# intelligent-machine-learning/dlrover

Hardware: AMD Instinct MI355X
Metric: checkpoint save+restore sec and goodput % under injected failure, Llama-3-8B FSDP 1/2/4/8 MI355X (higher is better)
Workload: dtype bf16; 1 GPU; model=llama3_8b, params=8030261248, global_batch=2, seq_len=4096, parallelism=fsdp1, ckpt_interval=2, ckpt_scope=full, ckpt_restored_step=1

## Files before the change

### dlrover_amd/ops/csrc/attention_bwd_v3.hip

```cpp
#include <cstdlib>
#include "kern_common.h"

typedef __attribute__((ext_vector_type(8))) __bf16 bf16x8;
typedef __attribute__((ext_vector_type(16))) float f32x16_t;
typedef __attribute__((ext_vector_type(2))) unsigned int u32x2_t;
typedef __attribute__((ext_vector_type(4))) unsigned int u32x4_t;
typedef __attribute__((ext_vector_type(2))) __bf16 bf16x2;

#define FB_D 128
#define FB_QB 256
#define FB_T 64

__device__ __forceinline__ int swzb(int row, int byte_col) {
  return byte_col ^ ((row & 7) << 4);
}

__device__ __forceinline__ unsigned pk_bf16(float lo, float hi) {
  bf16x2 v = {(__bf16)lo, (__bf16)hi};
  return *reinterpret_cast<unsigned*>(&v);
}

__device__ __forceinline__ bf16x8 trT_frag(const char* lds, int rb, int n,
                                           int lane, int half) {
  const int j = (lane & 15) >> 2;
  const int dq = n * 8 + ((lane & 16) >> 2) + (lane & 3);
  const int r0 = rb + half * 8 + j;
  const int r1 = r0 + 4;
  const unsigned base = (unsigned)(uintptr_t)lds;
  const unsigned a0 = base + r0 * 256 + ((dq * 8) ^ ((r0 & 7) << 4));
  const unsigned a1 = base + r1 * 256 + ((dq * 8) ^ ((r1 & 7) << 4));
  u32x2_t w0, w1;
  asm volatile(
      "ds_read_b64_tr_b16 %0, %2\n\t"
      "ds_read_b64_tr_b16 %1, %3\n\t"
      "s_waitcnt lgkmcnt(0)"
      : "=v"(w0), "=v"(w1)
      : "v"(a0), "v"(a1));
  u32x4_t frag = u32x4_t{w0.x, w0.y, w1.x, w1.y};
  return *reinterpret_cast<bf16x8*>(&frag);
}

__device__ __forceinline__ void pairswap_frags(const float v16[16], int half,
                                               bf16x8 out[2]) {
#pragma unroll
  for (int ks2 = 0; ks2 < 2; ++ks2) {
    const int r0 = ks2 * 8;
    unsigned w0 = pk_bf16(v16[r0 + 0], v16[r0 + 1]);
    unsigned w1 = pk_bf16(v16[r0 + 2], v16[r0 + 3]);
    unsigned w2 = pk_bf16(v16[r0 + 4], v16[r0 + 5]);
    unsigned w3 = pk_bf16(v16[r0 + 6], v16[r0 + 7]);
    u32x2_t s0 = __builtin_amdgcn_permlane32_swap(w0, w2, false, false);
    u32x2_t s1 = __builtin_amdgcn_permlane32_swap(w1, w3, false, false);
    u32x4_t frag = u32x4_t{s0.x, s1.x, s0.y, s1.y};
    out[ks2] = *reinterpret_cast<bf16x8*>(&frag);
  }
  (void)half;
}


__global__ __launch_bounds__(512) void fa_bwd_dq_v3_kernel(
    const short* __restrict__ q, const short* __restrict__ k,
    const short* __restrict__ v, const short* __restrict__ dout,
    const float* __restrict__ lse, const float* __restrict__ dvec,
    short* __restrict__ dq, int B, int H, int HKV, int S, float scale,
    long long qs_b, long long qs_h, long long qs_s,
    long long ks_b, long long ks_h, long long ks_s,
    long long vs_b, long long vs_h, long long vs_s,
    long long ds_b, long long ds_h, long long ds_s) {
  __shared__ char k_lds[2][FB_T * FB_D * 2];
  __shared__ char v_lds[2][FB_T * FB_D * 2];

  const int tid = threadIdx.x;
  const int wave = tid >> 6;
  const int lane = tid & 63;
  const int half = lane >> 5;
  const int qcol = lane & 31;

  const int qt = blockIdx.x;
  const int h = blockIdx.y;
  const int b = blockIdx.z;
  const int g = h / (H / HKV);

  const short* q_blk = q + (long long)b * qs_b + (long long)h * qs_h +
                       (long long)(qt * FB_QB) * qs_s;
  const short* do_blk = dout + (long long)b * ds_b + (long long)h * ds_h +
                        (long long)(qt * FB_QB) * ds_s;
  const short* k_head = k + (long long)b * ks_b + (long long)g * ks_h;
  const short* v_head = v + (long long)b * vs_b + (long long)g * vs_h;

  const int q_row_w = wave * 32 + qcol;
  const int q_glob = qt * FB_QB + q_row_w;

  bf16x8 bq[8], bdo[8];
#pragma unroll
  for (int ks = 0; ks < 8; ++ks) {
    bq[ks] = *reinterpret_cast<const bf16x8*>(
        q_blk + (long long)q_row_w * qs_s + ks * 16 + half * 8);
    bdo[ks] = *reinterpret_cast<const bf16x8*>(
        do_blk + (long long)q_row_w * ds_s + ks * 16 + half * 8);
  }
  const long long lrow = ((long long)b * H + h) * S + q_glob;
  const float L = lse[lrow];
  const float Dv = dvec[lrow];

  f32x16_t acc_dq[4];
#pragma unroll
  for (int n = 0; n < 4; ++n)
#pragma unroll
    for (int r = 0; r < 16; ++r) acc_dq[n][r] = 0.f;

  bf16x8 st_k[2], st_v[2];
  const int st_row0 = (tid * 16) / FB_D;
  const int st_col0 = (tid * 16) % FB_D;
  auto issue_loads = [&](int kt) {
    const short* ksrc = k_head + (long long)(kt * FB_T) * ks_s;
    const short* vsrc = v_head + (long long)(kt * FB_T) * vs_s;
#pragma unroll
    for (int c = 0; c < 2; ++c) {
      st_k[c] = *reinterpret_cast<const bf16x8*>(
          ksrc + (long long)st_row0 * ks_s + st_col0 + c * 8);
      st_v[c] = *reinterpret_cast<const bf16x8*>(
          vsrc + (long long)st_row0 * vs_s + st_col0 + c * 8);
    }
  };
  auto write_lds = [&](int buf) {
#pragma unroll
    for (int c = 0; c < 2; ++c) {
      const int col = st_col0 + c * 8;
      *reinterpret_cast<bf16x8*>(k_lds[buf] + st_row0 * 256 +
                                 swzb(st_row0, col * 2)) = st_k[c];
      *reinterpret_cast<bf16x8*>(v_lds[buf] + st_row0 * 256 +
                                 swzb(st_row0, col * 2)) = st_v[c];
    }
  };

  const int n_tiles = (qt + 1) * (FB_QB / FB_T);
  const int wave_q_max = qt * FB_QB + wave * 32 + 31;

  issue_loads(0);
  write_lds(0);
  __syncthreads();

  for (int kt = 0; kt < n_tiles; ++kt) {
    const int cur = kt & 1;
    const char* k_cur = k_lds[cur];
    const char* v_cur = v_lds[cur];
    if (kt + 1 < n_tiles) issue_loads(kt + 1);

    const int kv0 = kt * FB_T;
    if (kv0 <= wave_q_max) {
      bf16x8 bds[4];
#pragma unroll
      for (int n = 0; n < 2; ++n) {
        f32x16_t acc_s;
#pragma unroll
        for (int r = 0; r < 16; ++r) acc_s[r] = 0.f;
#pragma unroll
        for (int ks = 0; ks < 8; ++ks) {
          const int row = n * 32 + qcol;
          bf16x8 ak = *reinterpret_cast<const bf16x8*>(
              k_cur + row * 256 + swzb(row, (ks * 16 + half * 8) * 2));
          acc_s = __builtin_amdgcn_mfma_f32_32x32x16_bf16(ak, bq[ks], acc_s,
                                                          0, 0, 0);
        }
#pragma unroll
        for (int r = 0; r < 16; ++r) {
          const int kv_glob = kv0 + n * 32 + (r & 3) + 8 * (r >> 2) + 4 * half;
          acc_s[r] =
              (kv_glob > q_glob) ? 0.f : __expf(acc_s[r] * scale - L);
        }
        f32x16_t acc_dp;
#pragma unroll
        for (int r = 0; r < 16; ++r) acc_dp[r] = 0.f;
#pragma unroll
        for (int ks = 0; ks < 8; ++ks) {
          const int row = n * 32 + qcol;
          bf16x8 av = *reinterpret_cast<const bf16x8*>(
              v_cur + row * 256 + swzb(row, (ks * 16 + half * 8) * 2));
          acc_dp = __builtin_amdgcn_mfma_f32_32x32x16_bf16(av, bdo[ks],
                                                           acc_dp, 0, 0, 0);
        }
        float dsv[16];
#pragma unroll
        for (int r = 0; r < 16; ++r)
          dsv[r] = acc_s[r] * (acc_dp[r] - Dv) * scale;
        pairswap_frags(dsv, half, &bds[n * 2]);
      }
#pragma unroll
      for (int n = 0; n < 4; ++n) {
#pragma unroll
        for (int ks = 0; ks < 4; ++ks) {
          bf16x8 akT = trT_frag(k_cur, ks * 16, n, lane, half);
          acc_dq[n] = __builtin_amdgcn_mfma_f32_32x32x16_bf16(
              akT, bds[ks], acc_dq[n], 0, 0, 0);
        }
      }
    }

    __syncthreads();
    if (kt + 1 < n_tiles) {
      write_lds(cur ^ 1);
      __syncthreads();
    }
  }

  short* dq_blk = dq + (long long)b * qs_b + (long long)h * qs_h +
                  (long long)(qt * FB_QB) * qs_s;
  char* slab = (char*)k_lds + (wave & 3) * (32 * FB_D * 2);
  for (int round = 0; round < 2; ++round) {
    __syncthreads();
    if ((wave >> 2) == round) {
#pragma unroll
      for (int n = 0; n < 4; ++n) {
#pragma unroll
        for (int r = 0; r < 16; ++r) {
          const int d = n * 32 + (r & 3) + 8 * (r >> 2) + 4 * half;
          *reinterpret_cast<__bf16*>(slab + qcol * 256 + swzb(qcol, d * 2)) =
              (__bf16)acc_dq[n][r];
        }
      }
    }
    __syncthreads();
    if ((wave >> 2) == round) {
#pragma unroll
      for (int pass = 0; pass < 4; ++pass) {
        const int elem0 = (pass * 64 + lane) * 16;
        const int r2 = elem0 / FB_D;
        const int c2 = elem0 % FB_D;
        bf16x8 v0 = *reinterpret_cast<const bf16x8*>(
            slab + r2 * 256 + swzb(r2, c2 * 2));
        bf16x8 v1 = *reinterpret_cast<const bf16x8*>(
            slab + r2 * 256 + swzb(r2, (c2 + 8) * 2));
        short* dst = dq_blk + (long long)(wave * 32 + r2) * qs_s + c2;
        *reinterpret_cast<bf16x8*>(dst) = v0;
        *reinterpret_cast<bf16x8*>(dst + 8) = v1;
      }
    }
  }
}


#define FB_DKV_PROLOGUE()                                                    \
  __shared__ char q_lds[FB_T * FB_D * 2];                                    \
  __shared__ char do_lds[FB_T * FB_D * 2];                                   \
  __shared__ float l_lds[FB_T];                                              \
  __shared__ float d_lds[FB_T];                                              \
  const int tid = threadIdx.x;                                               \
  const int wave = tid >> 6;                                                 \
  const int lane = tid & 63;                                                 \
  const int half = lane >> 5;                                                \
  const int kcol = lane & 31;                                                \
  const int kvb0 = blockIdx.x * FB_QB;                                       \
  const int chunk = blockIdx.y;                                              \
  const int CH = gridDim.y;                                                  \
  const int bg = blockIdx.z;                                                 \
  const int b = bg / HKV;                                                    \
  const int g = bg % HKV;                                                    \
  const int rep = H / HKV;                                                   \
  const int kv_own = kvb0 + wave * 32 + kcol;                                \
  const short* k_head = k + (long long)b * ks_b + (long long)g * ks_h;       \
  bf16x8 bk[8];                                                              \
  _Pragma("unroll") for (int ks = 0; ks < 8; ++ks) bk[ks] =                  \
      *reinterpret_cast<const bf16x8*>(k_head + (long long)kv_own * ks_s +   \
                                       ks * 16 + half * 8);                  \
  const int qt_min = kvb0 / FB_T;                                            \
  const int n_qt = S / FB_T - qt_min;                                        \
  const int n_work = rep * n_qt;                                             \
  const int wave_kv_min = kvb0 + wave * 32;                                  \
  auto stage_qdo = [&](int h, int qt) {                                      \
    const short* qsrc = q + (long long)b * qs_b + (long long)h * qs_h +      \
                        (long long)(qt * FB_T) * qs_s;                       \
    const short* dsrc = dout + (long long)b * ds_b + (long long)h * ds_h +   \
                        (long long)(qt * FB_T) * ds_s;                       \
    _Pragma("unroll") for (int c = 0; c < 2; ++c) {                          \
      const int linear = (tid * 16) + c * 8;                                 \
      const int row = linear / FB_D;                                         \
      const int col = linear % FB_D;                                         \
      *reinterpret_cast<bf16x8*>(q_lds + row * 256 + swzb(row, col * 2)) =   \
          *reinterpret_cast<const bf16x8*>(qsrc + (long long)row * qs_s +    \
                                           col);                             \
      *reinterpret_cast<bf16x8*>(do_lds + row * 256 + swzb(row, col * 2)) =  \
          *reinterpret_cast<const bf16x8*>(dsrc + (long long)row * ds_s +    \
                                           col);                             \
    }                                                                        \
    if (tid < FB_T) {                                                        \
      const long long lrow = ((long long)b * H + h) * S + qt * FB_T + tid;   \
      l_lds[tid] = lse[lrow];                                                \
      d_lds[tid] = dvec[lrow];                                               \
    }                                                                        \
  }

__global__ __launch_bounds__(512) void fa_bwd_dv_v3_kernel(
    const short* __restrict__ q, const short* __restrict__ k,
    const short* __restrict__ v, const short* __restrict__ dout,
    const float* __restrict__ lse, const float* __restrict__ dvec,
    float* __restrict__ dk32, float* __restrict__ dv32, int B, int H,
    int HKV, int S, float scale,
    long long qs_b, long long qs_h, long long qs_s,
    long long ks_b, long long ks_h, long long ks_s,
    long long vs_b, long long vs_h, long long vs_s,
    long long ds_b, long long ds_h, long long ds_s) {
  FB_DKV_PROLOGUE();

  {
    f32x16_t acc_dv[4];
#pragma unroll
    for (int n = 0; n < 4; ++n)
#pragma unroll
      for (int r = 0; r < 16; ++r) acc_dv[n][r] = 0.f;

    for (int w = chunk; w < n_work; w += CH) {
      const int h = g * rep + w / n_qt;
      const int qt = qt_min + w % n_qt;
      __syncthreads();
      stage_qdo(h, qt);
      __syncthreads();
      if (qt * FB_T + FB_T - 1 < wave_kv_min) continue;
#pragma unroll
      for (int st = 0; st < 2; ++st) {
        const int q0 = qt * FB_T + st * 32;
        if (q0 + 31 < wave_kv_min) continue;
        f32x16_t acc_s;
#pragma unroll
        for (int r = 0; r < 16; ++r) acc_s[r] = 0.f;
#pragma unroll
        for (int ks = 0; ks < 8; ++ks) {
          const int row = st * 32 + kcol;
          bf16x8 aq = *reinterpret_cast<const bf16x8*>(
              q_lds + (st * 32 + kcol) * 256 +
              swzb(st * 32 + kcol, (ks * 16 + half * 8) * 2));
          (void)row;
          acc_s = __builtin_amdgcn_mfma_f32_32x32x16_bf16(aq, bk[ks], acc_s,
                                                          0, 0, 0);
        }
        float pv[16];
#pragma unroll
        for (int r = 0; r < 16; ++r) {
          const int qrow = st * 32 + (r & 3) + 8 * (r >> 2) + 4 * half;
          const int q_glob = qt * FB_T + qrow;
          pv[r] = (kv_own > q_glob)
                      ? 0.f
                      : __expf(acc_s[r] * scale - l_lds[qrow]);
        }
        bf16x8 bp[2];
        pairswap_frags(pv, half, bp);
#pragma unroll
        for (int n = 0; n < 4; ++n) {
#pragma unroll
          for (int ks2 = 0; ks2 < 2; ++ks2) {
            bf16x8 adoT =
                trT_frag(do_lds, st * 32 + ks2 * 16, n, lane, half);
            acc_dv[n] = __builtin_amdgcn_mfma_f32_32x32x16_bf16(
                adoT, bp[ks2], acc_dv[n], 0, 0, 0);
          }
        }
      }
    }
    float* dv_base = dv32 + ((long long)bg * S + kv_own) * FB_D;
#pragma unroll
    for (int n = 0; n < 4; ++n)
// ... 140 lines not shown
```

### dlrover_amd/ops/csrc/bindings.cpp

```cpp
#include <torch/extension.h>
#include <ATen/cuda/CUDAContext.h>

#include <tuple>

extern "C" {
void rmsnorm_fwd_launch(const void*, const void*, void*, void*, int, int,
                        float, void*);
void rmsnorm_add_fwd_launch(const void*, const void*, const void*, void*,
                            void*, void*, int, int, float, void*);
void rmsnorm_bwd_launch(const void*, const void*, const void*, const void*,
                        const void*, void*, void*, void*, void*, int, int,
                        int, void*);
void rope_launch(void*, const void*, const void*, const void*, long long,
                 long long, int, int, int, void*);
void rope_oop_launch(const void*, void*, const void*, const void*,
                     const void*, long long, long long, int, int, long long,
                     int, void*);
void swiglu_fwd_launch(const void*, void*, long long, int, void*);
void swiglu_bwd_launch(const void*, const void*, void*, long long, int, void*);
void adamw_launch(void*, const void*, void*, void*, void*, long long, float,
                  float, float, float, float, int, int, float, void*);
void causal_softmax_fwd_launch(void*, long long, int, int, int, float, void*);
void causal_softmax_bwd_launch(void*, const void*, long long, int, float,
                               void*);
void cross_entropy_launch(void*, const void*, void*, long long, int, int,
                          float, int, void*);
void mfma16_probe_launch(const void*, const void*, void*, void*);
void mfma32_probe_launch(const void*, const void*, void*, void*);
void tr_b16_probe3_launch(void*, void*);
void tr_b16_probe_launch(void*, void*);
void flash_attn_fwd_launch(const void*, const void*, const void*, void*,
                           void*, int, int, int, int, float,
                           const long long*, void*);
void flash_attn_fwd_v3_launch(const void*, const void*, const void*, void*,
                              void*, int, int, int, int, float,
                              const long long*, void*);
void flash_attn_fwd_v2_launch(const void*, const void*, const void*, void*,
                              void*, int, int, int, int, float,
                              const long long*, void*);
void fa_bwd_pre_launch(const void*, const void*, void*, int, int, int,
                       const long long*, const long long*, void*);
void fa_bwd_dq_launch(const void*, const void*, const void*, const void*,
                      const void*, const void*, void*, int, int, int, int,
                      float, const long long*, void*);
void fa_bwd_dq_v3_launch(const void*, const void*, const void*, const void*,
                         const void*, const void*, void*, int, int, int, int,
                         float, const long long*, void*);
void fa_bwd_dkv_v3_launch(const void*, const void*, const void*, const void*,
                          const void*, const void*, void*, void*, int, int,
                          int, int, float, const long long*, void*);
void fa_bwd_dkv_launch(const void*, const void*, const void*, const void*,
                       const void*, const void*, void*, void*, int, int, int,
                       int, float, const long long*, void*);
void f32_to_bf16_launch(const void*, void*, long long, void*);
}

namespace {

void* cur_stream() {
  return (void*)at::cuda::getCurrentCUDAStream().stream();
}

void check_bf16(const at::Tensor& t, const char* name) {
  TORCH_CHECK(t.is_cuda(), name, " must be on GPU");
  TORCH_CHECK(t.is_contiguous(), name, " must be contiguous");
  TORCH_CHECK(t.scalar_type() == at::kBFloat16, name, " must be bf16");
}

std::tuple<at::Tensor, at::Tensor> rmsnorm_fwd(const at::Tensor& x,
                                               const at::Tensor& w,
                                               double eps) {
  check_bf16(x, "x");
  check_bf16(w, "w");
  const int hidden = (int)x.size(-1);
  TORCH_CHECK(hidden % 8 == 0, "hidden must be a multiple of 8");
  const long long n_rows = x.numel() / hidden;
  auto y = at::empty_like(x);
  auto invrms = at::empty({n_rows}, x.options().dtype(at::kFloat));
  rmsnorm_fwd_launch(x.data_ptr(), w.data_ptr(), y.data_ptr(),
                     invrms.data_ptr(), (int)n_rows, hidden, (float)eps,
                     cur_stream());
  return {y, invrms};
}

std::tuple<at::Tensor, at::Tensor, at::Tensor> rmsnorm_add_fwd(
    const at::Tensor& x, const at::Tensor& resid, const at::Tensor& w,
    double eps) {
  check_bf16(x, "x");
  check_bf16(resid, "resid");
  const int hidden = (int)x.size(-1);
  const long long n_rows = x.numel() / hidden;
  auto h = at::empty_like(x);
  auto y = at::empty_like(x);
  auto invrms = at::empty({n_rows}, x.options().dtype(at::kFloat));
  rmsnorm_add_fwd_launch(x.data_ptr(), resid.data_ptr(), w.data_ptr(),
                         h.data_ptr(), y.data_ptr(), invrms.data_ptr(),
                         (int)n_rows, hidden, (float)eps, cur_stream());
  return {h, y, invrms};
}

std::tuple<at::Tensor, at::Tensor> rmsnorm_bwd(
    const at::Tensor& dy, const at::Tensor& x, const at::Tensor& w,
    const at::Tensor& invrms, c10::optional<at::Tensor> dh_extra) {
  check_bf16(dy, "dy");
  check_bf16(x, "x");
  const int hidden = (int)x.size(-1);
  TORCH_CHECK(hidden <= 16384, "rmsnorm_bwd: hidden > 16384 unsupported "
              "(register dw accumulator: RMSN_MAX_VPT)");
  const long long n_rows = x.numel() / hidden;
  const int n_partials = (int)(n_rows < 2048 ? (n_rows > 0 ? n_rows : 1) : 2048);
  auto dx = at::empty_like(x);
  auto dw = at::empty_like(w);
  auto partial =
      at::empty({n_partials, hidden}, x.options().dtype(at::kFloat));
  auto dw_f32 = at::zeros({hidden}, x.options().dtype(at::kFloat));
  const void* dh_ptr = nullptr;
  if (dh_extra.has_value()) {
    check_bf16(*dh_extra, "dh_extra");
    dh_ptr = dh_extra->data_ptr();
  }
  rmsnorm_bwd_launch(dy.data_ptr(), x.data_ptr(), w.data_ptr(),
                     invrms.data_ptr(), dh_ptr, dx.data_ptr(),
                     partial.data_ptr(), dw_f32.data_ptr(), dw.data_ptr(),
                     (int)n_rows, hidden, n_partials, cur_stream());
  return {dx, dw};
}

void rope_apply(at::Tensor& x, const at::Tensor& pos, const at::Tensor& cos,
                const at::Tensor& sin, bool backward) {
  check_bf16(x, "x");
  TORCH_CHECK(pos.scalar_type() == at::kInt && pos.is_cuda(),
              "pos must be int32 on GPU");
  TORCH_CHECK(cos.scalar_type() == at::kFloat && cos.is_contiguous(),
              "cos table must be contiguous fp32");
  const int head_dim = (int)x.size(-1);
  const int n_heads = (int)x.size(-2);
  TORCH_CHECK(head_dim % 8 == 0, "head_dim must be a multiple of 8");
  const long long n_tokens = x.numel() / ((long long)n_heads * head_dim);
  TORCH_CHECK(pos.numel() > 0 && n_tokens % pos.numel() == 0,
              "pos length must divide the token count (one entry per "
              "sequence position)");
  rope_launch(x.data_ptr(), pos.data_ptr(), cos.data_ptr(), sin.data_ptr(),
              n_tokens, (long long)pos.numel(), n_heads, head_dim,
              backward ? 1 : 0, cur_stream());
}

at::Tensor rope_rotate_oop(const at::Tensor& x, const at::Tensor& pos,
                           const at::Tensor& cos, const at::Tensor& sin,
                           bool backward) {
  TORCH_CHECK(x.is_cuda(), "x must be on GPU");
  TORCH_CHECK(x.scalar_type() == at::kBFloat16, "x must be bf16");
  TORCH_CHECK(pos.scalar_type() == at::kInt && pos.is_cuda(),
              "pos must be int32 on GPU");
  const int head_dim = (int)x.size(-1);
  const int n_heads = (int)x.size(-2);
  TORCH_CHECK(head_dim % 8 == 0, "head_dim must be a multiple of 8");
  TORCH_CHECK(x.stride(-1) == 1 && x.stride(-2) == head_dim,
              "rope: head_dim/heads must be contiguous within a token row");
  const long long n_tokens = x.numel() / ((long long)n_heads * head_dim);
  long long tok_stride = n_heads * (long long)head_dim;
  if (x.dim() >= 3) {
    tok_stride = x.stride(-3);
    long long rows = x.size(-3);
    for (int d = (int)x.dim() - 4; d >= 0; --d) {
      TORCH_CHECK(x.stride(d) == rows * tok_stride,
                  "rope: leading dims must be uniformly strided");
      rows *= x.size(d);
    }
  }
  TORCH_CHECK(pos.numel() > 0 && n_tokens % pos.numel() == 0,
              "pos length must divide the token count");
  auto out = at::empty(x.sizes(), x.options());
  rope_oop_launch(x.data_ptr(), out.data_ptr(), pos.data_ptr(),
                  cos.data_ptr(), sin.data_ptr(), n_tokens,
                  (long long)pos.numel(), n_heads, head_dim, tok_stride,
                  backward ? 1 : 0, cur_stream());
  return out;
}

at::Tensor swiglu_fwd(const at::Tensor& gate_up) {
  check_bf16(gate_up, "gate_up");
  const int two_inner = (int)gate_up.size(-1);
  TORCH_CHECK(two_inner % 16 == 0, "inner dim must be a multiple of 8");
  const int inner = two_inner / 2;
  const long long n_rows = gate_up.numel() / two_inner;
  auto sizes = gate_up.sizes().vec();
  sizes.back() = inner;
  auto out = at::empty(sizes, gate_up.options());
  swiglu_fwd_launch(gate_up.data_ptr(), out.data_ptr(), n_rows, inner,
                    cur_stream());
  return out;
}

at::Tensor swiglu_bwd(const at::Tensor& dy, const at::Tensor& gate_up) {
  check_bf16(dy, "dy");
  check_bf16(gate_up, "gate_up");
  const int inner = (int)gate_up.size(-1) / 2;
  const long long n_rows = gate_up.numel() / (2LL * inner);
  auto d_gate_up = at::empty_like(gate_up);
  swiglu_bwd_launch(dy.data_ptr(), gate_up.data_ptr(), d_gate_up.data_ptr(),
                    n_rows, inner, cur_stream());
  return d_gate_up;
}

void adamw_step(at::Tensor& param, const at::Tensor& grad, at::Tensor& m,
                at::Tensor& v, c10::optional<at::Tensor> param_bf16,
                double lr, double beta1, double beta2, double eps,
                double weight_decay, int64_t step, double grad_scale) {
  TORCH_CHECK(param.scalar_type() == at::kFloat && param.is_contiguous(),
              "master param must be contiguous fp32");
  TORCH_CHECK(grad.is_cuda() && grad.is_contiguous(), "grad must be GPU");
  TORCH_CHECK(grad.numel() == param.numel(), "grad/param numel mismatch");
  const bool gbf16 = grad.scalar_type() == at::kBFloat16;
  TORCH_CHECK(gbf16 || grad.scalar_type() == at::kFloat,
              "grad must be bf16 or fp32");
  void* pb = nullptr;
  if (param_bf16.has_value()) {
    check_bf16(*param_bf16, "param_bf16");
    pb = param_bf16->data_ptr();
  }
  adamw_launch(param.data_ptr(), grad.data_ptr(), m.data_ptr(), v.data_ptr(),
               pb, param.numel(), (float)lr, (float)beta1, (float)beta2,
               (float)eps, (float)weight_decay, (int)step, gbf16 ? 1 : 0,
               (float)grad_scale, cur_stream());
}

void causal_softmax_fwd(at::Tensor& scores, int64_t q_len, int64_t q_offset,
                        double scale) {
  check_bf16(scores, "scores");
  const int row_len = (int)scores.size(-1);
  TORCH_CHECK(row_len % 8 == 0, "row_len must be a multiple of 8");
  const long long n_rows = scores.numel() / row_len;
  causal_softmax_fwd_launch(scores.data_ptr(), n_rows, row_len, (int)q_len,
                            (int)q_offset, (float)scale, cur_stream());
}

void causal_softmax_bwd(at::Tensor& dscores, const at::Tensor& probs,
                        double scale) {
  check_bf16(dscores, "dscores");
  check_bf16(probs, "probs");
  const int row_len = (int)dscores.size(-1);
  const long long n_rows = dscores.numel() / row_len;
  causal_softmax_bwd_launch(dscores.data_ptr(), probs.data_ptr(), n_rows,
                            row_len, (float)scale, cur_stream());
}

static void check_attn_view(const at::Tensor& t, const char* name) {
  TORCH_CHECK(t.is_cuda() && t.scalar_type() == at::kBFloat16, name,
              " must be bf16 GPU");
  TORCH_CHECK(t.dim() == 4 && t.stride(3) == 1, name,
              " must be [B,H,S,D] with contiguous D");
}

static void pack_strides(long long* st, const at::Tensor& t, int at) {
  st[at + 0] = (long long)t.stride(0);
  st[at + 1] = (long long)t.stride(1);
  st[at + 2] = (long long)t.stride(2);
}

std::tuple<at::Tensor, at::Tensor> flash_attn_fwd(const at::Tensor& q,
                                                  const at::Tensor& k,
                                                  const at::Tensor& v,
                                                  double scale) {
  check_attn_view(q, "q");
  check_attn_view(k, "k");
  check_attn_view(v, "v");
  const int B = (int)q.size(0), H = (int)q.size(1), S = (int)q.size(2);
  const int D = (int)q.size(3), HKV = (int)k.size(1);
  TORCH_CHECK(D == 128, "flash_attn: head_dim must be 128");
  TORCH_CHECK(S % 64 == 0, "flash_attn: seq len must be a multiple of 64");
  TORCH_CHECK(H % HKV == 0, "flash_attn: H % HKV != 0");
  auto out_bshd = at::empty({B, S, H, D}, q.options());
  auto out = out_bshd.permute({0, 2, 1, 3});
  auto lse = at::empty({B, H, S}, q.options().dtype(at::kFloat));
  long long st[12];
  pack_strides(st, q, 0);
  pack_strides(st, k, 3);
  pack_strides(st, v, 6);
  pack_strides(st, out, 9);
  static const bool use_v2 = []() {
    const char* e = getenv("DLROVER_FA_V2");
    return e != nullptr && e[0] == '1';
  }();
  static const bool v3_enabled = []() {
    const char* e = getenv("DLROVER_FA_V3");
    return e == nullptr || e[0] != '0';
  }();
  if (v3_enabled && !use_v2 && S % 256 == 0) {
    flash_attn_fwd_v3_launch(q.data_ptr(), k.data_ptr(), v.data_ptr(),
                             out_bshd.data_ptr(), lse.data_ptr(), B, H, HKV,
                             S, (float)scale, st, cur_stream());
  } else if (use_v2) {
    flash_attn_fwd_v2_launch(q.data_ptr(), k.data_ptr(), v.data_ptr(),
                             out_bshd.data_ptr(), lse.data_ptr(), B, H, HKV,
                             S, (float)scale, st, cur_stream());
  } else {
    flash_attn_fwd_launch(q.data_ptr(), k.data_ptr(), v.data_ptr(),
                          out_bshd.data_ptr(), lse.data_ptr(), B, H, HKV, S,
                          (float)scale, st, cur_stream());
  }
  return {out, lse};
}

std::tuple<at::Tensor, at::Tensor, at::Tensor> flash_attn_bwd(
    const at::Tensor& q, const at::Tensor& k, const at::Tensor& v,
    const at::Tensor& out, const at::Tensor& dout_in, const at::Tensor& lse,
    double scale) {
  check_attn_view(q, "q");
  check_attn_view(k, "k");
  check_attn_view(v, "v");
  const int B = (int)q.size(0), H = (int)q.size(1), S = (int)q.size(2);
  const int D = (int)q.size(3), HKV = (int)k.size(1);
  at::Tensor dout = dout_in;
  if (dout.strides() != out.strides()) {
    dout = at::empty_like(out.permute({0, 2, 1, 3}).contiguous())
               .view({B, S, H, D});
    dout = dout.permute({0, 2, 1, 3});
    dout.copy_(dout_in);
  }
  TORCH_CHECK(dout.stride(3) == 1, "dout needs contiguous D");
  auto dvec = at::empty({B, H, S}, q.options().dtype(at::kFloat));
  {
    long long ost[3], dstr[3];
    pack_strides(ost, out, 0);
    pack_strides(dstr, dout, 0);
    fa_bwd_pre_launch(dout.data_ptr(), out.data_ptr(), dvec.data_ptr(), B, H,
                      S, ost, dstr, cur_stream());
    long long st[12];
    pack_strides(st, q, 0);
    pack_strides(st, k, 3);
    pack_strides(st, v, 6);
    pack_strides(st, dout, 9);
    auto dq_bshd = at::empty({B, S, H, D}, q.options());
    auto dq = dq_bshd.permute({0, 2, 1, 3});
    {
      long long stq[12];
      pack_strides(stq, dq, 0);
      pack_strides(stq, k, 3);
      pack_strides(stq, v, 6);
      pack_strides(stq, dout, 9);
      at::Tensor quse = q;
      if (q.strides() != dq.strides()) {
        auto q_bshd = at::empty({B, S, H, D}, q.options());
        auto qv = q_bshd.permute({0, 2, 1, 3});
        qv.copy_(q);
        quse = qv;
        pack_strides(stq, quse, 0);
      }
      static const bool bwd_v3 = []() {
        const char* e = getenv("DLROVER_FA_BWD_V3");
        return e == nullptr || e[0] != '0';
      }();
      auto dk32 = at::zeros({B, HKV, S, D}, k.options().dtype(at::kFloat));
      auto dv32 = at::zeros({B, HKV, S, D}, v.options().dtype(at::kFloat));
      if (bwd_v3 && S % 256 == 0) {
        fa_bwd_dq_v3_launch(quse.data_ptr(), k.data_ptr(), v.data_ptr(),
                            dout.data_ptr(), lse.data_ptr(), dvec.data_ptr(),
                            dq_bshd.data_ptr(), B, H, HKV, S, (float)scale,
                            stq, cur_stream());
        fa_bwd_dkv_v3_launch(quse.data_ptr(), k.data_ptr(), v.data_ptr(),
                             dout.data_ptr(), lse.data_ptr(),
                             dvec.data_ptr(), dk32.data_ptr(),
                             dv32.data_ptr(), B, H, HKV, S, (float)scale,
                             stq, cur_stream());
      } else {
        fa_bwd_dq_launch(quse.data_ptr(), k.data_ptr(), v.data_ptr(),
                         dout.data_ptr(), lse.data_ptr(), dvec.data_ptr(),
                         dq_bshd.data_ptr(), B, H, HKV, S, (float)scale, stq,
                         cur_stream());
        fa_bwd_dkv_launch(quse.data_ptr(), k.data_ptr(), v.data_ptr(),
                          dout.data_ptr(), lse.data_ptr(), dvec.data_ptr(),
                          dk32.data_ptr(), dv32.data_ptr(), B, H, HKV, S,
                          (float)scale, stq, cur_stream());
      }
      auto dk = at::empty({B, HKV, S, D}, k.options());
      auto dv = at::empty({B, HKV, S, D}, v.options());
      f32_to_bf16_launch(dk32.data_ptr(), dk.data_ptr(), dk32.numel(),
                         cur_stream());
      f32_to_bf16_launch(dv32.data_ptr(), dv.data_ptr(), dv32.numel(),
                         cur_stream());
      return {dq, dk, dv};
    }
  }
}

at::Tensor mfma16_probe(const at::Tensor& A, const at::Tensor& B) {
  check_bf16(A, "A");
  check_bf16(B, "B");
  TORCH_CHECK(A.sizes() == at::IntArrayRef({16, 32}) &&
              B.sizes() == at::IntArrayRef({32, 16}),
              "probe wants A[16,32], B[32,16]");
  auto C = at::empty({16, 16}, A.options().dtype(at::kFloat));
  mfma16_probe_launch(A.data_ptr(), B.data_ptr(), C.data_ptr(), cur_stream());
  return C;
}

void memcpy_d2h_async(int64_t dst_addr, const at::Tensor& src) {
  TORCH_CHECK(src.is_cuda() && src.is_contiguous(), "src must be cuda+contig");
  auto err = hipMemcpyAsync((void*)dst_addr, src.data_ptr(), src.nbytes(),
                            hipMemcpyDeviceToHost,
                            (hipStream_t)cur_stream());
  TORCH_CHECK(err == hipSuccess, "hipMemcpyAsync D2H: ", hipGetErrorString(err));
}

void memcpy_h2d_async(at::Tensor& dst, int64_t src_addr, int64_t nbytes) {
  TORCH_CHECK(dst.is_cuda() && dst.is_contiguous(), "dst must be cuda+contig");
  TORCH_CHECK(nbytes <= (int64_t)dst.nbytes(), "overflow");
  auto err = hipMemcpyAsync(dst.data_ptr(), (const void*)src_addr, nbytes,
                            hipMemcpyHostToDevice,
                            (hipStream_t)cur_stream());
  TORCH_CHECK(err == hipSuccess, "hipMemcpyAsync H2D: ", hipGetErrorString(err));
}

at::Tensor mfma32_probe(const at::Tensor& A, const at::Tensor& B) {
  check_bf16(A, "A");
  check_bf16(B, "B");
  TORCH_CHECK(A.sizes() == at::IntArrayRef({32, 16}) &&
              B.sizes() == at::IntArrayRef({16, 32}),
              "probe wants A[32,16], B[16,32]");
  auto C = at::empty({32, 32}, A.options().dtype(at::kFloat));
  mfma32_probe_launch(A.data_ptr(), B.data_ptr(), C.data_ptr(), cur_stream());
  return C;
}

at::Tensor cross_entropy_fwd_bwd(at::Tensor& logits, const at::Tensor& targets,
                                 int64_t ignore_index, double grad_scale,
                                 bool compute_grad) {
  check_bf16(logits, "logits");
  TORCH_CHECK(targets.scalar_type() == at::kInt && targets.is_cuda(),
              "targets must be int32 on GPU");
  const int vocab = (int)logits.size(-1);
  const long long n_rows = logits.numel() / vocab;
  TORCH_CHECK(targets.numel() == n_rows, "one target per row");
  auto losses = at::empty({n_rows}, logits.options().dtype(at::kFloat));
  cross_entropy_launch(logits.data_ptr(), targets.data_ptr(),
                       losses.data_ptr(), n_rows, vocab, (int)ignore_index,
                       (float)grad_scale, compute_grad ? 1 : 0, cur_stream());
  return losses;
}

}

PYBIND11_MODULE(TORCH_EXTENSION_NAME, m) {
  m.doc() = "dlrover_amd CDNA4 (gfx950) kernels";
  m.def("rmsnorm_fwd", &rmsnorm_fwd, "fused RMSNorm forward (bf16)");
  m.def("rmsnorm_bwd", &rmsnorm_bwd, "fused RMSNorm backward (bf16)");
  m.def("rmsnorm_add_fwd", &rmsnorm_add_fwd,
        "fused residual-add + RMSNorm forward -> (h, y, invrms)");
  m.def("rope_apply", &rope_apply, "in-place RoPE rotate-half (bf16)");
  m.def("rope_rotate_oop", &rope_rotate_oop,
        "out-of-place RoPE: strided source -> contiguous output");
  m.def("swiglu_fwd", &swiglu_fwd, "fused SwiGLU forward (bf16)");
  m.def("swiglu_bwd", &swiglu_bwd, "fused SwiGLU backward (bf16)");
  m.def("adamw_step", &adamw_step, "fused AdamW with fp32 master weights");
  m.def("causal_softmax_fwd", &causal_softmax_fwd,
        "in-place fused scale+causal-mask+softmax (bf16)");
  m.def("causal_softmax_bwd", &causal_softmax_bwd,
        "in-place softmax backward (bf16)");
  m.def("cross_entropy_fwd_bwd", &cross_entropy_fwd_bwd,
        "fused CE loss + in-place dlogits (bf16)");
  m.def("tr_b16_probe", []() {
    auto out = at::empty({64, 12}, at::TensorOptions()
                                      .dtype(at::kBFloat16)
                                      .device(at::kCUDA));
    tr_b16_probe_launch(out.data_ptr(), cur_stream());
    return out;
  }, "ds_read_b64_tr_b16 semantics probe");
  m.def("mfma16_probe", &mfma16_probe, "MFMA 16x16x32 bf16 layout self-test");
  m.def("mfma32_probe", &mfma32_probe, "MFMA 32x32x16 bf16 layout self-test");
  m.def("memcpy_d2h_async", &memcpy_d2h_async,
        "hipMemcpyAsync device tensor -> registered host address");
  m.def("memcpy_h2d_async", &memcpy_h2d_async,
        "hipMemcpyAsync registered host address -> device tensor");
  m.def("tr_b16_probe3", []() {
    auto out = at::empty({64, 12}, at::TensorOptions()
                                      .dtype(at::kShort)
                                      .device(at::kCUDA));
    tr_b16_probe3_launch(out.data_ptr(), cur_stream());
    return out;
  }, "tr_b16 cooperative tile-sourcing probe (raw index bits)");
  m.def("flash_attn_fwd", &flash_attn_fwd,
        "flash attention forward (bf16, causal, GQA, D=128) -> (out, lse)");
  m.def("flash_attn_bwd", &flash_attn_bwd,
        "flash attention backward -> (dq, dk, dv)");
}
```

### setup.py

```python

import os

from setuptools import setup

os.environ.setdefault("PYTORCH_ROCM_ARCH", "gfx950")

from torch.utils.cpp_extension import BuildExtension, CUDAExtension

ROOT = os.path.dirname(os.path.abspath(__file__))
CSRC = os.path.join(ROOT, "dlrover_amd", "ops", "csrc")

sources = [
    os.path.join(CSRC, "bindings.cpp"),
    os.path.join(CSRC, "rmsnorm.hip"),
    os.path.join(CSRC, "rope.hip"),
    os.path.join(CSRC, "swiglu.hip"),
    os.path.join(CSRC, "adamw.hip"),
    os.path.join(CSRC, "softmax.hip"),
    os.path.join(CSRC, "cross_entropy.hip"),
    os.path.join(CSRC, "mfma_probe.hip"),
    os.path.join(CSRC, "attention.hip"),
    os.path.join(CSRC, "attention_v3.hip"),
    os.path.join(CSRC, "attention_bwd.hip"),
    os.path.join(CSRC, "attention_bwd_v3.hip"),
]

setup(
    name="dlrover_amd_ops",
    ext_modules=[
        CUDAExtension(
            name="dlrover_amd.ops._hip_ops",
            sources=sources,
            extra_compile_args={
                "cxx": ["-O3", "-std=c++17"],
                "nvcc": ["-O3", "-std=c++17", "--offload-arch=gfx950"],
            },
        )
    ],
    cmdclass={"build_ext": BuildExtension.with_options(use_ninja=True)},
)
```

Measured before the change: 60.07 goodput_percent.

## Add v4 flash-attention dK/dV backward kernel with balanced chunking and direct bf16 output

Adds a new dK/dV backward kernel that splits work across blocks in load-balanced chunks sized to the CU count. It double-buffers Q/dO tiles in LDS and writes bf16 dK/dV directly when a key block is not chunked, which avoids the fp32 zero-init, atomics and conversion pass in that case. Chunked key blocks still use fp32 atomics plus a conversion kernel. The code becomes the default through a new variant argument, and the shared fragment helpers move into a common header. The metric is checkpoint goodput, so changes in backward attention time may barely show up in it.

```diff
diff --git a/dlrover_amd/ops/csrc/attention_bwd_v3.hip b/dlrover_amd/ops/csrc/attention_bwd_v3.hip
--- a/dlrover_amd/ops/csrc/attention_bwd_v3.hip
+++ b/dlrover_amd/ops/csrc/attention_bwd_v3.hip
@@ -1,61 +1,5 @@
 #include <cstdlib>
-#include "kern_common.h"
-
-typedef __attribute__((ext_vector_type(8))) __bf16 bf16x8;
-typedef __attribute__((ext_vector_type(16))) float f32x16_t;
-typedef __attribute__((ext_vector_type(2))) unsigned int u32x2_t;
-typedef __attribute__((ext_vector_type(4))) unsigned int u32x4_t;
-typedef __attribute__((ext_vector_type(2))) __bf16 bf16x2;
-
-#define FB_D 128
-#define FB_QB 256
-#define FB_T 64
-
-__device__ __forceinline__ int swzb(int row, int byte_col) {
-  return byte_col ^ ((row & 7) << 4);
-}
-
-__device__ __forceinline__ unsigned pk_bf16(float lo, float hi) {
-  bf16x2 v = {(__bf16)lo, (__bf16)hi};
-  return *reinterpret_cast<unsigned*>(&v);
-}
-
-__device__ __forceinline__ bf16x8 trT_frag(const char* lds, int rb, int n,
-                                           int lane, int half) {
-  const int j = (lane & 15) >> 2;
-  const int dq = n * 8 + ((lane & 16) >> 2) + (lane & 3);
-  const int r0 = rb + half * 8 + j;
-  const int r1 = r0 + 4;
-  const unsigned base = (unsigned)(uintptr_t)lds;
-  const unsigned a0 = base + r0 * 256 + ((dq * 8) ^ ((r0 & 7) << 4));
-  const unsigned a1 = base + r1 * 256 + ((dq * 8) ^ ((r1 & 7) << 4));
-  u32x2_t w0, w1;
-  asm volatile(
-      "ds_read_b64_tr_b16 %0, %2\n\t"
-      "ds_read_b64_tr_b16 %1, %3\n\t"
-      "s_waitcnt lgkmcnt(0)"
-      : "=v"(w0), "=v"(w1)
-      : "v"(a0), "v"(a1));
-  u32x4_t frag = u32x4_t{w0.x, w0.y, w1.x, w1.y};
-  return *reinterpret_cast<bf16x8*>(&frag);
-}
-
-__device__ __forceinline__ void pairswap_frags(const float v16[16], int half,
-                                               bf16x8 out[2]) {
-#pragma unroll
-  for (int ks2 = 0; ks2 < 2; ++ks2) {
-    const int r0 = ks2 * 8;
-    unsigned w0 = pk_bf16(v16[r0 + 0], v16[r0 + 1]);
-    unsigned w1 = pk_bf16(v16[r0 + 2], v16[r0 + 3]);
-    unsigned w2 = pk_bf16(v16[r0 + 4], v16[r0 + 5]);
-    unsigned w3 = pk_bf16(v16[r0 + 6], v16[r0 + 7]);
-    u32x2_t s0 = __builtin_amdgcn_permlane32_swap(w0, w2, false, false);
-    u32x2_t s1 = __builtin_amdgcn_permlane32_swap(w1, w3, false, false);
-    u32x4_t frag = u32x4_t{s0.x, s1.x, s0.y, s1.y};
-    out[ks2] = *reinterpret_cast<bf16x8*>(&frag);
-  }
-  (void)half;
-}
+#include "fa_bwd_frag.h"
 
 
 __global__ __launch_bounds__(512) void fa_bwd_dq_v3_kernel(
diff --git a/dlrover_amd/ops/csrc/attention_bwd_v4.hip b/dlrover_amd/ops/csrc/attention_bwd_v4.hip
--- /dev/null
+++ b/dlrover_amd/ops/csrc/attention_bwd_v4.hip
@@ -0,0 +1,337 @@
+#include "fa_bwd_frag.h"
+
+#define F4_QDO_BYTES (2 * 2 * FB_T * FB_D * 2)
+#define F4_VIMG_BYTES (FB_QB * FB_D * 2)
+#define F4_LD_BYTES (2 * 2 * FB_T * 4)
+#define F4_SMEM (F4_QDO_BYTES + F4_VIMG_BYTES + F4_LD_BYTES)
+#define F4_NUM_CU 256
+#define F4_MIN_UNITS 8
+
+__host__ __device__ __forceinline__ int f4_nch(int n_work, int T) {
+  return (n_work + T - 1) / T;
+}
+
+static int f4_units_per_item(int B, int H, int HKV, int S) {
+  const int rep = H / HKV;
+  long long total = 0;
+  for (int kb = 0; kb < S / FB_QB; ++kb)
+    total += (long long)rep * (S / FB_T - kb * (FB_QB / FB_T));
+  total *= (long long)B * HKV;
+  long long T = (total + 2 * F4_NUM_CU - 1) / (2 * F4_NUM_CU);
+  return T < F4_MIN_UNITS ? F4_MIN_UNITS : (int)T;
+}
+
+__device__ __forceinline__ int f4_slab_pos(int row, int d) {
+  return row * FB_D + (d ^ (row & 31) ^ (((d >> 2) & 1) << 5));
+}
+
+template <int OFF0, int OFF1>
+__device__ __forceinline__ bf16x8 f4_tr(unsigned addr) {
+  u32x2_t w0, w1;
+  asm volatile(
+      "ds_read_b64_tr_b16 %0, %2 offset:%3\n\t"
+      "ds_read_b64_tr_b16 %1, %2 offset:%4\n\t"
+      "s_waitcnt lgkmcnt(0)"
+      : "=&v"(w0), "=&v"(w1)
+      : "v"(addr), "n"(OFF0), "n"(OFF1));
+  u32x4_t frag = u32x4_t{w0.x, w0.y, w1.x, w1.y};
+  return *reinterpret_cast<bf16x8*>(&frag);
+}
+
+template <int ST>
+__device__ __forceinline__ void f4_accum(unsigned tile, const bf16x8 (&bp)[2],
+                                         const bf16x8 (&bds)[2],
+                                         f32x16_t (&acc_dv)[4],
+                                         f32x16_t (&acc_dk)[4]) {
+#define F4_STEP(N, KS2)                                                      \
+  {                                                                          \
+    constexpr int o0 = (ST * 32 + KS2 * 16) * 256 + N * 64;                  \
+    constexpr int o1 = (ST * 32 + KS2 * 16) * 256 + (N ^ 1) * 64 + 1024;     \
+    constexpr int dO = FB_T * FB_D * 2;                                      \
+    bf16x8 adoT = f4_tr<o0 + dO, o1 + dO>(tile);                             \
+    acc_dv[N] = __builtin_amdgcn_mfma_f32_32x32x16_bf16(adoT, bp[KS2],       \
+                                                        acc_dv[N], 0, 0, 0); \
+    bf16x8 aqT = f4_tr<o0, o1>(tile);                                        \
+    acc_dk[N] = __builtin_amdgcn_mfma_f32_32x32x16_bf16(aqT, bds[KS2],       \
+                                                        acc_dk[N], 0, 0, 0); \
+  }
+  F4_STEP(0, 0) F4_STEP(0, 1) F4_STEP(1, 0) F4_STEP(1, 1)
+  F4_STEP(2, 0) F4_STEP(2, 1) F4_STEP(3, 0) F4_STEP(3, 1)
+#undef F4_STEP
+}
+
+__global__ __launch_bounds__(512) void fa_bwd_dkv_v4_kernel(
+    const short* __restrict__ q, const short* __restrict__ k,
+    const short* __restrict__ v, const short* __restrict__ dout,
+    const float* __restrict__ lse, const float* __restrict__ dvec,
+    float* __restrict__ dk32, float* __restrict__ dv32,
+    short* __restrict__ dk, short* __restrict__ dv, int B, int H, int HKV,
+    int S, float scale, int T,
+    long long qs_b, long long qs_h, long long qs_s,
+    long long ks_b, long long ks_h, long long ks_s,
+    long long vs_b, long long vs_h, long long vs_s,
+    long long ds_b, long long ds_h, long long ds_s) {
+  __shared__ __attribute__((aligned(16))) char smem[F4_SMEM];
+  char* const qdo_lds = smem;
+  char* const v_img = smem + F4_QDO_BYTES;
+  float* const ld_lds =
+      reinterpret_cast<float*>(smem + F4_QDO_BYTES + F4_VIMG_BYTES);
+
+  const int tid = threadIdx.x;
+  const int wave = tid >> 6;
+  const int lane = tid & 63;
+  const int half = lane >> 5;
+  const int kcol = lane & 31;
+
+  const int rep = H / HKV;
+  const int BG = B * HKV;
+  const int nkb = S / FB_QB;
+  int idx = blockIdx.x, kb = 0, nch = 1;
+  for (; kb < nkb; ++kb) {
+    nch = f4_nch(rep * (S / FB_T - kb * (FB_QB / FB_T)), T);
+    const int cnt = nch * BG;
+    if (idx < cnt) break;
+    idx -= cnt;
+  }
+  if (kb >= nkb) return;
+  const int chunk = idx / BG;
+  const int bg = idx % BG;
+  const int b = bg / HKV;
+  const int g = bg % HKV;
+  const int kvb0 = kb * FB_QB;
+  const int kv_own = kvb0 + wave * 32 + kcol;
+  const int qt_min = kvb0 / FB_T;
+  const int n_qt = S / FB_T - qt_min;
+  const int n_work = rep * n_qt;
+  const int wave_kv_min = kvb0 + wave * 32;
+  const int tr_j = (lane & 15) >> 2;
+  const int tr_dql = ((lane & 16) >> 2) + (lane & 3);
+  const unsigned tr_lane_off =
+      (half * 8 + tr_j) * 256 + ((tr_dql * 8) ^ (tr_j << 4));
+
+  const short* k_head = k + (long long)b * ks_b + (long long)g * ks_h;
+  bf16x8 bk[8];
+#pragma unroll
+  for (int ks = 0; ks < 8; ++ks)
+    bk[ks] = *reinterpret_cast<const bf16x8*>(
+        k_head + (long long)kv_own * ks_s + ks * 16 + half * 8);
+
+  {
+    const short* v_rows = v + (long long)b * vs_b + (long long)g * vs_h +
+                          (long long)wave_kv_min * vs_s;
+#pragma unroll
+    for (int i = 0; i < 8; ++i) {
+      const int linear = (i * 64 + lane) * 8;
+      const int row = linear / FB_D;
+      const int col = linear % FB_D;
+      *reinterpret_cast<bf16x8*>(v_img + (wave * 32 + row) * 256 +
+                                 swzb(row, col * 2)) =
+          *reinterpret_cast<const bf16x8*>(v_rows + (long long)row * vs_s +
+                                           col);
+    }
+  }
+  const char* const v_wave = v_img + wave * 32 * 256;
+  int rd_off[4];
+#pragma unroll
+  for (int i = 0; i < 4; ++i)
+    rd_off[i] = kcol * 256 + swzb(kcol, (i * 16 + half * 8) * 2);
+
+  f32x16_t acc_dv[4], acc_dk[4];
+#pragma unroll
+  for (int n = 0; n < 4; ++n)
+#pragma unroll
+    for (int r = 0; r < 16; ++r) acc_dv[n][r] = acc_dk[n][r] = 0.f;
+
+  bf16x8 st_x[2];
+  float st_c = 0.f;
+  const int st_row = tid >> 3;
+  const int st_col = (tid & 7) * 16;
+  auto issue_loads = [&](int w, int which) {
+    const int h = g * rep + w / n_qt;
+    const int qt = qt_min + w % n_qt;
+    const short* src =
+        which ? dout + (long long)b * ds_b + (long long)h * ds_h +
+                    (long long)(qt * FB_T + st_row) * ds_s + st_col
+              : q + (long long)b * qs_b + (long long)h * qs_h +
+                    (long long)(qt * FB_T + st_row) * qs_s + st_col;
+#pragma unroll
+    for (int c = 0; c < 2; ++c)
+      st_x[c] = *reinterpret_cast<const bf16x8*>(src + c * 8);
+    if (tid < FB_T) {
+      const long long lrow = ((long long)b * H + h) * S + qt * FB_T + tid;
+      st_c = which ? dvec[lrow] : lse[lrow];
+    }
+  };
+  auto commit_lds = [&](int buf, int which) {
+    char* xb = qdo_lds + (buf * 2 + which) * (FB_T * FB_D * 2);
+#pragma unroll
+    for (int c = 0; c < 2; ++c)
+      *reinterpret_cast<bf16x8*>(
+          xb + st_row * 256 + swzb(st_row, (st_col + c * 8) * 2)) = st_x[c];
+    if (tid < FB_T)
+      ld_lds[(buf * 2 + which) * FB_T + tid] = st_c;
+  };
+
+  issue_loads(chunk, 0);
+  commit_lds(0, 0);
+  issue_loads(chunk, 1);
+  commit_lds(0, 1);
+  __syncthreads();
+
+  int cur = 0;
+  for (int w = chunk; w < n_work; w += nch) {
+    const int qt = qt_min + w % n_qt;
+    const bool more = w + nch < n_work;
+
+    const char* q_lds = qdo_lds + cur * (2 * FB_T * FB_D * 2);
+    const char* do_lds = q_lds + FB_T * FB_D * 2;
+    const float* l_lds = ld_lds + cur * 2 * FB_T;
+    const float* d_lds = l_lds + FB_T;
+
+    const bool live = qt * FB_T + FB_T - 1 >= wave_kv_min;
+#pragma unroll
+    for (int st = 0; st < 2; ++st) {
+      if (more) issue_loads(w + nch, st);
+      const int q0 = qt * FB_T + st * 32;
+      if (live && q0 + 31 >= wave_kv_min) {
+        f32x16_t acc_s, acc_dp;
+#pragma unroll
+        for (int r = 0; r < 16; ++r) acc_s[r] = acc_dp[r] = 0.f;
+#pragma unroll
+        for (int ks = 0; ks < 8; ++ks) {
+          const int ro = rd_off[ks & 3] + (ks >> 2) * 128;
+          bf16x8 aq = *reinterpret_cast<const bf16x8*>(
+              q_lds + st * (32 * 256) + ro);
+          acc_s = __builtin_amdgcn_mfma_f32_32x32x16_bf16(aq, bk[ks], acc_s,
+                                                          0, 0, 0);
+          bf16x8 ado = *reinterpret_cast<const bf16x8*>(
+              do_lds + st * (32 * 256) + ro);
+          bf16x8 bv = *reinterpret_cast<const bf16x8*>(v_wave + ro);
+          acc_dp = __builtin_amdgcn_mfma_f32_32x32x16_bf16(ado, bv, acc_dp,
+                                                           0, 0, 0);
+        }
+        float pv[16], dsv[16];
+#pragma unroll
+        for (int r = 0; r < 16; ++r) {
+          const int qrow = st * 32 + (r & 3) + 8 * (r >> 2) + 4 * half;
+          const int q_glob = qt * FB_T + qrow;
+          const float p = (kv_own > q_glob)
+                              ? 0.f
+                              : __expf(acc_s[r] * scale - l_lds[qrow]);
+          pv[r] = p;
+          dsv[r] = p * (acc_dp[r] - d_lds[qrow]) * scale;
+        }
+        bf16x8 bp[2], bds[2];
+        pairswap_frags(pv, half, bp);
+        pairswap_frags(dsv, half, bds);
+        const unsigned tile = (unsigned)(uintptr_t)q_lds + tr_lane_off;
+        if (st == 0)
+          f4_accum<0>(tile, bp, bds, acc_dv, acc_dk);
+        else
+          f4_accum<1>(tile, bp, bds, acc_dv, acc_dk);
+      }
+      if (more) commit_lds(cur ^ 1, st);
+    }
+    __syncthreads();
+    cur ^= 1;
+  }
+
+  int elane = lane;
+  asm volatile("" : "+v"(elane));
+  const int ekcol = elane & 31;
+  const int ehalf = elane >> 5;
+  float* slab = reinterpret_cast<float*>(smem) + wave * (32 * FB_D);
+  const long long orow0 = (long long)b * S + wave_kv_min;
+  const bool direct = nch == 1;
+#pragma unroll
+  for (int which = 0; which < 2; ++which) {
+    if (which) __syncthreads();
+#pragma unroll
+    for (int n = 0; n < 4; ++n)
+#pragma unroll
+      for (int r = 0; r < 16; ++r) {
+        const int d = n * 32 + (r & 3) + 8 * (r >> 2) + 4 * ehalf;
+        slab[f4_slab_pos(ekcol, d)] = which ? acc_dv[n][r] : acc_dk[n][r];
+      }
+    __syncthreads();
+    if (direct) {
+      short* dst = which ? dv : dk;
+#pragma unroll
+      for (int i = 0; i < 8; ++i) {
+        const int t = i * 64 + elane;
+        const int row = t >> 4;
+        const int d0 = (t & 15) * 8;
+        u32x4_t pk;
+#pragma unroll
+        for (int e = 0; e < 4; ++e)
+          pk[e] = pk_bf16(slab[f4_slab_pos(row, d0 + 2 * e)],
+                          slab[f4_slab_pos(row, d0 + 2 * e + 1)]);
+        *reinterpret_cast<u32x4_t*>(
+            dst + ((orow0 + row) * HKV + g) * FB_D + d0) = pk;
+      }
+    } else {
+      float* dst = which ? dv32 : dk32;
+#pragma unroll 4
+      for (int row = 0; row < 32; ++row) {
+        float* drow = dst + ((orow0 + row) * HKV + g) * FB_D;
+#pragma unroll
+        for (int j = 0; j < 2; ++j) {
+          const int d = j * 64 + elane;
+          unsafeAtomicAdd(drow + d, slab[f4_slab_pos(row, d)]);
+        }
+      }
+    }
+  }
+}
+
+__global__ __launch_bounds__(256) void fa_bwd_v4_cvt_kernel(
+    const float* __restrict__ dk32, const float* __restrict__ dv32,
+    short* __restrict__ dk, short* __restrict__ dv, int H, int HKV, int S,
+    int T, long long n8) {
+  const long long i = (long long)blockIdx.x * 256 + threadIdx.x;
+  if (i >= n8) return;
+  const float* src = blockIdx.y ? dv32 : dk32;
+  short* dst = blockIdx.y ? dv : dk;
+  const int key = (int)((i * 8 / ((long long)HKV * FB_D)) % S);
+  const int kb = key / FB_QB;
+  if (f4_nch((H / HKV) * (S / FB_T - kb * (FB_QB / FB_T)), T) == 1) return;
+  const float4_t a = *reinterpret_cast<const float4_t*>(src + i * 8);
+  const float4_t c = *reinterpret_cast<const float4_t*>(src + i * 8 + 4);
+  u32x4_t pk = {pk_bf16(a[0], a[1]), pk_bf16(a[2], a[3]),
+                pk_bf16(c[0], c[1]), pk_bf16(c[2], c[3])};
+  *reinterpret_cast<u32x4_t*>(dst + i * 8) = pk;
+}
+
+extern "C" int fa_bwd_dkv_v4_chunked(int B, int H, int HKV, int S) {
+  const int T = f4_units_per_item(B, H, HKV, S);
+  return f4_nch((H / HKV) * (S / FB_T), T) > 1;
+}
+
+extern "C" void fa_bwd_dkv_v4_launch(const void* q, const void* k,
+                                     const void* v, const void* dout,
+                                     const void* lse, const void* dvec,
+                                     void* dk32, void* dv32, void* dk,
+                                     void* dv, int B, int H, int HKV, int S,
+                                     float scale, const long long* strides,
+                                     hipStream_t stream) {
+  const int T = f4_units_per_item(B, H, HKV, S);
+  const int rep = H / HKV;
+  int items = 0;
+  for (int kb = 0; kb < S / FB_QB; ++kb)
+    items += f4_nch(rep * (S / FB_T - kb * (FB_QB / FB_T)), T) * B * HKV;
+  hipLaunchKernelGGL(fa_bwd_dkv_v4_kernel, dim3(items), dim3(512), 0, stream,
+                     (const short*)q, (const short*)k, (const short*)v,
+                     (const short*)dout, (const float*)lse,
+                     (const float*)dvec, (float*)dk32, (float*)dv32,
+                     (short*)dk, (short*)dv, B, H, HKV, S, scale, T,
+                     strides[0], strides[1], strides[2], strides[3],
+                     strides[4], strides[5], strides[6], strides[7],
+                     strides[8], strides[9], strides[10], strides[11]);
+  if (fa_bwd_dkv_v4_chunked(B, H, HKV, S)) {
+    const long long n8 = (long long)B * S * HKV * FB_D / 8;
+    dim3 grid((unsigned)((n8 + 255) / 256), 2);
+    hipLaunchKernelGGL(fa_bwd_v4_cvt_kernel, grid, dim3(256), 0, stream,
+                       (const float*)dk32, (const float*)dv32, (short*)dk,
+                       (short*)dv, H, HKV, S, T, n8);
+  }
+}
diff --git a/dlrover_amd/ops/csrc/bindings.cpp b/dlrover_amd/ops/csrc/bindings.cpp
--- a/dlrover_amd/ops/csrc/bindings.cpp
+++ b/dlrover_amd/ops/csrc/bindings.cpp
@@ -49,6 +49,11 @@
 void fa_bwd_dkv_v3_launch(const void*, const void*, const void*, const void*,
                           const void*, const void*, void*, void*, int, int,
                           int, int, float, const long long*, void*);
+void fa_bwd_dkv_v4_launch(const void*, const void*, const void*, const void*,
+                          const void*, const void*, void*, void*, void*,
+                          void*, int, int, int, int, float, const long long*,
+                          void*);
+int fa_bwd_dkv_v4_chunked(int, int, int, int);
 void fa_bwd_dkv_launch(const void*, const void*, const void*, const void*,
                        const void*, const void*, void*, void*, int, int, int,
                        int, float, const long long*, void*);
@@ -305,7 +310,9 @@
 std::tuple<at::Tensor, at::Tensor, at::Tensor> flash_attn_bwd(
     const at::Tensor& q, const at::Tensor& k, const at::Tensor& v,
     const at::Tensor& out, const at::Tensor& dout_in, const at::Tensor& lse,
-    double scale) {
+    double scale, int64_t variant) {
+  TORCH_CHECK(variant == 4 || variant == 3 || variant == 1,
+              "flash_attn_bwd: variant must be 4, 3 or 1");
   check_attn_view(q, "q");
   check_attn_view(k, "k");
   check_attn_view(v, "v");
@@ -347,13 +354,31 @@
         quse = qv;
         pack_strides(stq, quse, 0);
       }
-      static const bool bwd_v3 = []() {
-        const char* e = getenv("DLROVER_FA_BWD_V3");
-        return e == nullptr || e[0] != '0';
-      }();
+      if (variant == 4 && S % 256 == 0) {
+        fa_bwd_dq_v3_launch(quse.data_ptr(), k.data_ptr(), v.data_ptr(),
+                            dout.data_ptr(), lse.data_ptr(), dvec.data_ptr(),
+                            dq_bshd.data_ptr(), B, H, HKV, S, (float)scale,
+                            stq, cur_stream());
+        auto dkv = at::empty({2, B, S, HKV, D}, k.options());
+        at::Tensor dkv32;
+        float* dk32p = nullptr;
+        float* dv32p = nullptr;
+        if (fa_bwd_dkv_v4_chunked(B, H, HKV, S)) {
+          dkv32 = at::zeros({2, B, S, HKV, D}, k.options().dtype(at::kFloat));
+          dk32p = dkv32.data_ptr<float>();
+          dv32p = dk32p + dkv32.stride(0);
+        }
+        fa_bwd_dkv_v4_launch(quse.data_ptr(), k.data_ptr(), v.data_ptr(),
+                             dout.data_ptr(), lse.data_ptr(),
+                             dvec.data_ptr(), dk32p, dv32p,
+                             dkv[0].data_ptr(), dkv[1].data_ptr(), B, H, HKV,
+                             S, (float)scale, stq, cur_stream());
+        return {dq, dkv[0].permute({0, 2, 1, 3}),
+                dkv[1].permute({0, 2, 1, 3})};
+      }
       auto dk32 = at::zeros({B, HKV, S, D}, k.options().dtype(at::kFloat));
       auto dv32 = at::zeros({B, HKV, S, D}, v.options().dtype(at::kFloat));
-      if (bwd_v3 && S % 256 == 0) {
+      if (variant >= 3 && S % 256 == 0) {
         fa_bwd_dq_v3_launch(quse.data_ptr(), k.data_ptr(), v.data_ptr(),
                             dout.data_ptr(), lse.data_ptr(), dvec.data_ptr(),
                             dq_bshd.data_ptr(), B, H, HKV, S, (float)scale,
@@ -482,5 +507,9 @@
   m.def("flash_attn_fwd", &flash_attn_fwd,
         "flash attention forward (bf16, causal, GQA, D=128) -> (out, lse)");
   m.def("flash_attn_bwd", &flash_attn_bwd,
-        "flash attention backward -> (dq, dk, dv)");
-}
+        "flash attention backward -> (dq, dk, dv); variant 4 (default) / 3 / "
+        "1 selects the kernel generation per call",
+        py::arg("q"), py::arg("k"), py::arg("v"), py::arg("out"),
+        py::arg("dout"), py::arg("lse"), py::arg("scale"),
+        py::arg("variant") = 4);
+}
diff --git a/dlrover_amd/ops/csrc/fa_bwd_frag.h b/dlrover_amd/ops/csrc/fa_bwd_frag.h
--- /dev/null
+++ b/dlrover_amd/ops/csrc/fa_bwd_frag.h
@@ -0,0 +1,58 @@
+#pragma once
+#include "kern_common.h"
+
+typedef __attribute__((ext_vector_type(8))) __bf16 bf16x8;
+typedef __attribute__((ext_vector_type(16))) float f32x16_t;
+typedef __attribute__((ext_vector_type(2))) unsigned int u32x2_t;
+typedef __attribute__((ext_vector_type(4))) unsigned int u32x4_t;
+typedef __attribute__((ext_vector_type(2))) __bf16 bf16x2;
+
+#define FB_D 128
+#define FB_QB 256
+#define FB_T 64
+
+__device__ __forceinline__ int swzb(int row, int byte_col) {
+  return byte_col ^ ((row & 7) << 4);
+}
+
+__device__ __forceinline__ unsigned pk_bf16(float lo, float hi) {
+  bf16x2 v = {(__bf16)lo, (__bf16)hi};
+  return *reinterpret_cast<unsigned*>(&v);
+}
+
+__device__ __forceinline__ bf16x8 trT_frag(const char* lds, int rb, int n,
+                                           int lane, int half) {
+  const int j = (lane & 15) >> 2;
+  const int dq = n * 8 + ((lane & 16) >> 2) + (lane & 3);
+  const int r0 = rb + half * 8 + j;
+  const int r1 = r0 + 4;
+  const unsigned base = (unsigned)(uintptr_t)lds;
+  const unsigned a0 = base + r0 * 256 + ((dq * 8) ^ ((r0 & 7) << 4));
+  const unsigned a1 = base + r1 * 256 + ((dq * 8) ^ ((r1 & 7) << 4));
+  u32x2_t w0, w1;
+  asm volatile(
+      "ds_read_b64_tr_b16 %0, %2\n\t"
+      "ds_read_b64_tr_b16 %1, %3\n\t"
+      "s_waitcnt lgkmcnt(0)"
+      : "=&v"(w0), "=&v"(w1)
+      : "v"(a0), "v"(a1));
+  u32x4_t frag = u32x4_t{w0.x, w0.y, w1.x, w1.y};
+  return *reinterpret_cast<bf16x8*>(&frag);
+}
+
+__device__ __forceinline__ void pairswap_frags(const float v16[16], int half,
+                                               bf16x8 out[2]) {
+#pragma unroll
+  for (int ks2 = 0; ks2 < 2; ++ks2) {
+    const int r0 = ks2 * 8;
+    unsigned w0 = pk_bf16(v16[r0 + 0], v16[r0 + 1]);
+    unsigned w1 = pk_bf16(v16[r0 + 2], v16[r0 + 3]);
+    unsigned w2 = pk_bf16(v16[r0 + 4], v16[r0 + 5]);
+    unsigned w3 = pk_bf16(v16[r0 + 6], v16[r0 + 7]);
+    u32x2_t s0 = __builtin_amdgcn_permlane32_swap(w0, w2, false, false);
+    u32x2_t s1 = __builtin_amdgcn_permlane32_swap(w1, w3, false, false);
+    u32x4_t frag = u32x4_t{s0.x, s1.x, s0.y, s1.y};
+    out[ks2] = *reinterpret_cast<bf16x8*>(&frag);
+  }
+  (void)half;
+}
diff --git a/setup.py b/setup.py
--- a/setup.py
+++ b/setup.py
@@ -23,6 +23,7 @@
     os.path.join(CSRC, "attention_v3.hip"),
     os.path.join(CSRC, "attention_bwd.hip"),
     os.path.join(CSRC, "attention_bwd_v3.hip"),
+    os.path.join(CSRC, "attention_bwd_v4.hip"),
 ]
 
 setup(
```

Result: slower. 57.29 goodput_percent (-4.6%).
